# google/telluride_decoding

Hardware: AMD Instinct MI355X
Metric: TRF-fit samples/sec (higher is better)
Workload: dtype f32 (every product as 3 float16 products of a 2-piece split on the f16 MFMA, f32 accumulate, f64 slab sums; f64 solve)

## Files before the change

telluride_decoding_amd/csrc/lagcov.hip:

```cpp
#include <cstdlib>
#include <cstring>

#include "td_common.h"

namespace {

typedef float f32x16 __attribute__((ext_vector_type(16)));

constexpr int kThreads = 256;
constexpr int kTile = 128;
constexpr int kTileG = 64;
constexpr int kNpfU = 10;
constexpr int kNpfU2 = 13;
constexpr int kNpfG = 9;
constexpr int kLagsPerWg = 8;
constexpr int kHalo = 8;
constexpr size_t kLagcovScratchCap = size_t(256) << 20;

__device__ __forceinline__ int xcd_remap(int bid, int nwg) {
  const int q = nwg >> 3, r = nwg & 7;
  const int xcd = bid & 7, within = bid >> 3;
  const int base = xcd < r ? xcd * (q + 1) : r * (q + 1) + (xcd - r) * q;
  return base + within;
}

struct RowWindow {
  const float* base;
  int lo, hi;
  int ld, last;
};

__device__ __forceinline__ RowWindow row_window(const float* g, long long ld, long long row0,
                                                long long ut, long long valid, int c0, int c) {
  RowWindow rw;
  rw.base = g + (row0 + ut) * ld + c0;
  const long long lo = -ut, hi = valid - 1 - ut, lim = 1 << 20;
  rw.lo = (int)(lo < -lim ? -lim : (lo > lim ? lim : lo));
  rw.hi = (int)(hi < -lim ? -lim : (hi > lim ? lim : hi));
  rw.ld = (int)ld;
  rw.last = c - 1 - c0;
  return rw;
}

template <bool kVec4>
__device__ __forceinline__ float4 load_row4(const RowWindow& rw, int r, bool row_ok, int c4) {
  const int rc = max(rw.lo, min(r, rw.hi));
  const bool ok = row_ok && r >= rw.lo && r <= rw.hi;
  const float* p = rw.base + rc * rw.ld;
  float4 v;
  if (kVec4) {
    const bool ch_ok = c4 <= rw.last;
    v = *reinterpret_cast<const float4*>(p + (ch_ok ? c4 : 0));
    const bool k = ok && ch_ok;
    v.x = k ? v.x : 0.f; v.y = k ? v.y : 0.f; v.z = k ? v.z : 0.f; v.w = k ? v.w : 0.f;
  } else {
    const int last = rw.last;
    v.x = p[min(c4, last)]; v.y = p[min(c4 + 1, last)];
    v.z = p[min(c4 + 2, last)]; v.w = p[min(c4 + 3, last)];
    v.x = (ok && c4 + 0 <= last) ? v.x : 0.f;
    v.y = (ok && c4 + 1 <= last) ? v.y : 0.f;
    v.z = (ok && c4 + 2 <= last) ? v.z : 0.f;
    v.w = (ok && c4 + 3 <= last) ? v.w : 0.f;
  }
  return v;
}

template <bool kVec4>
__device__ __forceinline__ float4 load_row4_raw(const RowWindow& rw, int r, int c4) {
  const int rc = max(rw.lo, min(r, rw.hi));
  const float* p = rw.base + rc * rw.ld;
  float4 v;
  if (kVec4) {
    v = *reinterpret_cast<const float4*>(p + (c4 <= rw.last ? c4 : 0));
  } else {
    const int last = rw.last;
    v.x = p[min(c4, last)]; v.y = p[min(c4 + 1, last)];
    v.z = p[min(c4 + 2, last)]; v.w = p[min(c4 + 3, last)];
  }
  return v;
}

__device__ __forceinline__ float4 mask_row4(const RowWindow& rw, int r, bool row_ok, int c4, float4 v) {
  const bool ok = row_ok && r >= rw.lo && r <= rw.hi;
  v.x = (ok && c4 + 0 <= rw.last) ? v.x : 0.f;
  v.y = (ok && c4 + 1 <= rw.last) ? v.y : 0.f;
  v.z = (ok && c4 + 2 <= rw.last) ? v.z : 0.f;
  v.w = (ok && c4 + 3 <= rw.last) ? v.w : 0.f;
  return v;
}

template <bool kUnified, int kTileT, int kNPF, bool kVec4>
__device__ __forceinline__ void prefetch_tile(const LagParams& p, const LagWork& w, long long ut,
                                              int e0, int rows, int cat, int cbt, int tid,
                                              float4 (&pf)[kNPF]) {
  const int c4 = (tid & 15) * 4;
  const int r0 = tid >> 4;
  if (kUnified) {
    const RowWindow rw = row_window(p.a, p.lda, w.a_row0, ut, w.a_valid, cat * 64, p.ca);
#pragma unroll
    for (int i = 0; i < kNPF; ++i) {
      const int r = r0 + 16 * i;
      pf[i] = load_row4<kVec4>(rw, r, r < rows, c4);
    }
  } else {
    const RowWindow ra = row_window(p.a, p.lda, w.a_row0, ut, w.a_valid, cat * 64, p.ca);
    const RowWindow rb = row_window(p.b, p.ldb, w.b_row0, ut + e0, w.b_valid, cbt * 64, p.cb);
    const long long a_left = w.u_end - ut;
    const int a_lim = (int)(a_left < kTileT ? a_left : kTileT);
#pragma unroll
    for (int i = 0; i < kNPF; ++i) {
      const int r = r0 + 16 * i;
      if (16 * i + 15 < kTileT)
        pf[i] = load_row4<kVec4>(ra, r, r < a_lim, c4);
      else
        pf[i] = load_row4<kVec4>(rb, r - kTileT, r < rows, c4);
    }
  }
}

template <bool kUnified, int kTileT, int kNPF>
__device__ __forceinline__ void store_tile(float* lds, const LagWork& w, long long ut,
                                           int ones_col, int tid, float4 (&pf)[kNPF]) {
  const int c4 = (tid & 15) * 4;
#pragma unroll
  for (int i = 0; i < kNPF; ++i) {
    const int r = (tid >> 4) + 16 * i;
    float4 v = pf[i];
    if (!kUnified && 16 * i + 15 < kTileT && ones_col >= c4 && ones_col < c4 + 4) {
      const long long u = ut + r;
      const float one = (u >= w.u_begin && u < w.u_end) ? 1.f : 0.f;
      if (ones_col == c4) v.x = one;
      else if (ones_col == c4 + 1) v.y = one;
      else if (ones_col == c4 + 2) v.z = one;
      else v.w = one;
    }
    *reinterpret_cast<float4*>(lds + r * 64 + c4) = v;
  }
}

template <int kTileT, bool kM2, bool kN2>
__device__ __forceinline__ void mfma_tile(const float* __restrict__ as,
                                          const float* __restrict__ bs, int wave, int lane, int nk,
                                          f32x16 (&acc)[2][2][2]) {
  const int lr = lane & 31, lk = lane >> 5;
  const float* ap = as + lk * 64 + lr;
  const float* bp = bs + (lk + 2 * wave) * 64 + lr;
  auto ld = [&](int kk, float (&o)[6]) {
    o[0] = ap[kk * 128];
    o[1] = kM2 ? ap[kk * 128 + 32] : 0.f;
    o[2] = bp[kk * 128];
    o[3] = kN2 ? bp[kk * 128 + 32] : 0.f;
    o[4] = bp[kk * 128 + 64];
    o[5] = kN2 ? bp[kk * 128 + 96] : 0.f;
  };
  auto mm = [&](const float (&o)[6]) {
#pragma unroll
    for (int le = 0; le < 2; ++le) {
      const float b0 = o[2 + 2 * le], b1 = o[3 + 2 * le];
      acc[le][0][0] = __builtin_amdgcn_mfma_f32_32x32x2f32(o[0], b0, acc[le][0][0], 0, 0, 0);
      if (kM2) acc[le][1][0] = __builtin_amdgcn_mfma_f32_32x32x2f32(o[1], b0, acc[le][1][0], 0, 0, 0);
      if (kN2) {
        acc[le][0][1] = __builtin_amdgcn_mfma_f32_32x32x2f32(o[0], b1, acc[le][0][1], 0, 0, 0);
        if (kM2) acc[le][1][1] = __builtin_amdgcn_mfma_f32_32x32x2f32(o[1], b1, acc[le][1][1], 0, 0, 0);
      }
    }
  };
  const int nfull = nk >> 1;
  float c[6], n[6];
  ld(0, c);
  int kk = 0;
  for (; kk + 1 < nfull; kk += 2) {
    ld(kk + 1, n);
    mm(c);
    ld(kk + 2 < nfull ? kk + 2 : kk + 1, c);
    mm(n);
  }
  if (kk < nfull) mm(c);
  if (nk & 1) {
    ld(nfull, c);
    if (lk) { c[0] = 0.f; c[1] = 0.f; }
    mm(c);
  }
}

template <int kTileT, bool kM2, bool kN2>
__device__ __forceinline__ void mfma_tile_few(const float* __restrict__ as,
                                              const float* __restrict__ bs, int wave, int lane,
                                              int nk, int g, int lg, f32x16 (&acc)[2][2][2]) {
  const int lr = lane & 31, lk = lane >> 5;
  const int s_phases = 8 >> lg;
  const int nfull = nk >> 1;
#pragma unroll
  for (int le = 0; le < 2; ++le) {
    const int slot = 2 * wave + le;
    const int lag = slot & (g - 1), phase = slot >> lg;
    const float* ap = as + lk * 64 + lr;
    const float* bp = bs + (lk + lag) * 64 + lr;
    auto step = [&](int kk, bool tail) {
      const bool live = !tail || lk == 0;
      const float a0 = live ? ap[kk * 128] : 0.f;
      const float a1 = (kM2 && live) ? ap[kk * 128 + 32] : 0.f;
      const float b0 = bp[kk * 128];
      acc[le][0][0] = __builtin_amdgcn_mfma_f32_32x32x2f32(a0, b0, acc[le][0][0], 0, 0, 0);
      if (kM2) acc[le][1][0] = __builtin_amdgcn_mfma_f32_32x32x2f32(a1, b0, acc[le][1][0], 0, 0, 0);
      if (kN2) {
        const float b1 = bp[kk * 128 + 32];
        acc[le][0][1] = __builtin_amdgcn_mfma_f32_32x32x2f32(a0, b1, acc[le][0][1], 0, 0, 0);
        if (kM2) acc[le][1][1] = __builtin_amdgcn_mfma_f32_32x32x2f32(a1, b1, acc[le][1][1], 0, 0, 0);
      }
    };
#pragma unroll 4
    for (int kk = phase; kk < nfull; kk += s_phases) step(kk, false);
    if ((nk & 1) && (nfull & (s_phases - 1)) == phase) step(nfull, true);
  }
}

template <bool kUnified, int kTileT, int kNPF, bool kVec4, bool kFew>
__global__ __launch_bounds__(kThreads, 2) void lagcov_mfma_kernel(LagParams p) {
  extern __shared__ __attribute__((aligned(16))) float lds[];

  const int tid = threadIdx.x;
  const int lane = tid & 63;
  const int wave = __builtin_amdgcn_readfirstlane(tid >> 6);

  int id = xcd_remap(blockIdx.x, gridDim.x);
  const int group = id % p.n_groups; id /= p.n_groups;
  const int cbt = id % p.n_cbt; id /= p.n_cbt;
  const int cat = id % p.n_cat; id /= p.n_cat;
  const LagWork w = p.works[id];
  const int e0 = p.e_min + group * (kFew ? p.lag_g : kLagsPerWg);

  const int rows = kUnified ? kTileT + kHalo + e0 : 2 * kTileT + kHalo;
  const float* as = lds;
  const float* bs = kUnified ? lds + e0 * 64 : lds + kTileT * 64;

  const int ca_eff = p.ca + p.a_ones;
  const bool m2 = ca_eff - cat * 64 > 32;
  const bool n2 = p.cb - cbt * 64 > 32;
  const int ones_col = p.a_ones ? p.ca - cat * 64 : -1;

  f32x16 acc[2][2][2];
#pragma unroll
  for (int i = 0; i < 2; ++i)
#pragma unroll
    for (int j = 0; j < 2; ++j)
#pragma unroll
      for (int k = 0; k < 2; ++k)
#pragma unroll
        for (int r = 0; r < 16; ++r) acc[i][j][k][r] = 0.f;

  float4 pf[kNPF];
  prefetch_tile<kUnified, kTileT, kNPF, kVec4>(p, w, w.u_begin, e0, rows, cat, cbt, tid, pf);
  store_tile<kUnified, kTileT, kNPF>(lds, w, w.u_begin, ones_col, tid, pf);
  __syncthreads();

  for (long long ut = w.u_begin; ut < w.u_end; ut += kTileT) {
    const bool more = ut + kTileT < w.u_end;
    if (more)
      prefetch_tile<kUnified, kTileT, kNPF, kVec4>(p, w, ut + kTileT, e0, rows, cat, cbt, tid,
                                                      pf);
    const long long left = w.u_end - ut;
    const int nk = (kUnified && left < kTileT) ? (int)left : kTileT;
    if (kFew) {
      if (m2) {
        if (n2) mfma_tile_few<kTileT, true, true>(as, bs, wave, lane, nk, p.lag_g, p.lag_lg, acc);
        else    mfma_tile_few<kTileT, true, false>(as, bs, wave, lane, nk, p.lag_g, p.lag_lg, acc);
      } else {
        if (n2) mfma_tile_few<kTileT, false, true>(as, bs, wave, lane, nk, p.lag_g, p.lag_lg, acc);
        else    mfma_tile_few<kTileT, false, false>(as, bs, wave, lane, nk, p.lag_g, p.lag_lg, acc);
      }
    } else if (m2) {
      if (n2) mfma_tile<kTileT, true, true>(as, bs, wave, lane, nk, acc);
      else    mfma_tile<kTileT, true, false>(as, bs, wave, lane, nk, acc);
    } else {
      if (n2) mfma_tile<kTileT, false, true>(as, bs, wave, lane, nk, acc);
      else    mfma_tile<kTileT, false, false>(as, bs, wave, lane, nk, acc);
    }
    if (more) {
      __syncthreads();
      store_tile<kUnified, kTileT, kNPF>(lds, w, ut + kTileT, ones_col, tid, pf);
      __syncthreads();
    }
  }

  const int lr = lane & 31, lk = lane >> 5;
  float* slab = p.partial + (size_t)id * p.e_pad * p.ca_pad * p.cb_pad;
#pragma unroll
  for (int le = 0; le < 2; ++le) {
    int e_idx = group * kLagsPerWg + 2 * wave + le;
    if (kFew) {
      const int slot = 2 * wave + le;
      e_idx = ((slot >> p.lag_lg) * p.n_groups + group) * p.lag_g + (slot & (p.lag_g - 1));
    }
    float* pe = slab + (size_t)e_idx * p.ca_pad * p.cb_pad;
#pragma unroll
    for (int m = 0; m < 2; ++m)
#pragma unroll
      for (int n = 0; n < 2; ++n)
#pragma unroll
        for (int r = 0; r < 16; ++r) {
          const int i = cat * 64 + m * 32 + (r & 3) + 8 * (r >> 2) + 4 * lk;
          const int j = cbt * 64 + n * 32 + lr;
          pe[(size_t)i * p.cb_pad + j] = acc[le][m][n][r];
        }
  }
}

constexpr int kBfTile = 128;
template <int kRowDw, int kPieces> struct BfGeom {
  static constexpr int kRows = kRowDw == 83 ? 160 : 192;
  static constexpr int kPieceDw = 64 * kRowDw;
  static constexpr size_t kLdsBytes =
      sizeof(unsigned) * (2 * kPieces * kPieceDw + (kPieces == 2 ? 2 * 2 * 96 + 8 * 1024 : 0));
};
constexpr int kBfThreads = 512;

typedef td_u32x4 u32x4;

__device__ __forceinline__ float comp4(const float4& v, int q) {
  return q == 0 ? v.x : q == 1 ? v.y : q == 2 ? v.z : v.w;
}

template <bool kZero, int kBfPieceDw, bool kF16>
__device__ __forceinline__ void bf_kstep(const unsigned* __restrict__ ap,
                                         const unsigned* __restrict__ bp,
                                         const unsigned* a_mask, f32x16 (&acc)[4]) {
  constexpr int kP = kF16 ? 2 : 3;
  u32x4 a[kP];
  unsigned d[kP][6];
#pragma unroll
  for (int pc = 0; pc < kP; ++pc) {
#pragma unroll
    for (int i = 0; i < 4; ++i) a[pc][i] = ap[pc * kBfPieceDw + i];
#pragma unroll
    for (int i = 0; i < 6; ++i) d[pc][i] = bp[pc * kBfPieceDw + i];
  }
  if (a_mask) {
#pragma unroll
    for (int pc = 0; pc < kP; ++pc)
#pragma unroll
      for (int i = 0; i < 4; ++i) a[pc][i] &= a_mask[i];
  }
  u32x4 b[4][kP];
#pragma unroll
  for (int pc = 0; pc < kP; ++pc)
#pragma unroll
    for (int i = 0; i < 4; ++i) {
      b[0][pc][i] = d[pc][i];
      b[1][pc][i] = __builtin_amdgcn_alignbit(d[pc][i + 1], d[pc][i], 16);
      b[2][pc][i] = d[pc][i + 1];
      b[3][pc][i] = __builtin_amdgcn_alignbit(d[pc][i + 2], d[pc][i + 1], 16);
    }
  f32x16 c[4];
#pragma unroll
  for (int r = 0; r < 4; ++r) {
    if (kZero) {
#pragma unroll
      for (int k = 0; k < 16; ++k) c[r][k] = 0.f;
    } else {
      c[r] = acc[r];
    }
  }
  if constexpr (kF16) {
    constexpr int pa[3] = {1, 0, 0}, pb[3] = {0, 1, 0};
#pragma unroll
    for (int t = 0; t < 3; ++t)
#pragma unroll
      for (int r = 0; r < 4; ++r) c[r] = td_mfma_f16(a[pa[t] % kP], b[r][pb[t] % kP], c[r]);
  } else {
    constexpr int pa[6] = {2, 0, 1, 1, 0, 0}, pb[6] = {0, 2, 1, 0, 1, 0};
#pragma unroll
    for (int t = 0; t < 6; ++t)
#pragma unroll
      for (int r = 0; r < 4; ++r) c[r] = td_mfma_bf16(a[pa[t] % kP], b[r][pb[t] % kP], c[r]);
  }
#pragma unroll
  for (int r = 0; r < 4; ++r) acc[r] = c[r];
}

template <int kFrom, int kTo, int kBfPieceDw, bool kF16, int kChain>
__device__ __forceinline__ void bf_ksteps(const unsigned* __restrict__ ap,
                                          const unsigned* __restrict__ bp, f32x16 (&acc)[4],
                                          f32x16 (&total)[4]) {
#pragma unroll
  for (int s = kFrom; s < kTo; ++s) {
    if (s % kChain == 0) bf_kstep<true, kBfPieceDw, kF16>(ap + 8 * s, bp + 8 * s, nullptr, acc);
    else                 bf_kstep<false, kBfPieceDw, kF16>(ap + 8 * s, bp + 8 * s, nullptr, acc);
    if ((s + 1) % kChain == 0) {
#pragma unroll
      for (int r = 0; r < 4; ++r) total[r] += acc[r];
    }
    __builtin_amdgcn_sched_barrier(0);
  }
}

template <bool kVec4, int kBfRowDw, bool kF16, bool kVirt = false, bool kKs = false>
__global__ __launch_bounds__(kBfThreads) void lagcov_split_kernel(LagParams p) {
  static_assert(!kVirt || kF16, "virtual images: the float16 form");
  static_assert(!kKs || kVirt, "shared tasks: virtual images");
  constexpr int kChain = 8;
  constexpr int kP = kF16 ? 2 : 3;
  extern __shared__ __attribute__((aligned(16))) unsigned ldsu[];
  constexpr int kBfRows = BfGeom<kBfRowDw, kP>::kRows;
  constexpr int kBfPieceDw = BfGeom<kBfRowDw, kP>::kPieceDw;

  const int tid = threadIdx.x;
  const int lane = tid & 63;
  const int wave = __builtin_amdgcn_readfirstlane(tid >> 6);
  int quad = wave & 1, mt = (wave >> 1) & 1, nt = wave >> 2;

  int id = xcd_remap(blockIdx.x, gridDim.x);
  const int group = id % p.n_groups; id /= p.n_groups;
  const int part = id;
  LagWork w = p.works[id];
  const int e0 = group * kLagsPerWg;
  int lag_off = e0 + 4 * quad, out_lag = lag_off;
  bool active = true, a_ext = false;
  const VirtImage* img = nullptr;
  VirtSeg vs = {0, 0, 0};
  int kparts = 1, kq = 0;
  if constexpr (kVirt) {
    const VirtGroup* vg = p.vgroups + group;
    const VirtTask tk = vg->task[wave];
    img = p.vimgs + vg->image;
    mt = tk.mt; nt = tk.nt; lag_off = tk.lag0; out_lag = tk.out_lag;
    active = out_lag >= 0; a_ext = tk.a_ext != 0;
    if constexpr (kKs) {
      kparts = __builtin_amdgcn_readfirstlane((int)tk.kparts);
      kq = __builtin_amdgcn_readfirstlane((int)tk.kq);
    }
    vs = p.vsegs[id];
  }
  const int ksn = 8 / kparts, ks0 = kq * ksn;

  f32x16 total[4];
#pragma unroll
  for (int r = 0; r < 4; ++r)
#pragma unroll
    for (int k = 0; k < 16; ++k) total[r][k] = 0.f;

  const int c4 = (tid & 15) * 4, rg = tid >> 4;
  const bool has_tail = kBfRows == 192 || wave < 4;
  const bool early = wave < 4;
  float sc[4] = {1.f, 1.f, 1.f, 1.f};
  int vdesc[4] = {0, 0, 0, 0};
  if constexpr (kVirt) {
#pragma unroll
    for (int q = 0; q < 4; ++q) {
      const int k = kVec4 ? c4 + q : lane;
      vdesc[q] = (img->src[k] + 1) | (img->role[k] ? 0x100 : 0) | ((int)img->shift[k] << 16);
    }
  }
  constexpr int kVPairs = kBfRows / 16;
  auto v_src = [&](int q) { return (vdesc[q] & 0xff) - 1; };
  auto v_sh = [&](int q) { return vdesc[q] >> 16; };
  auto v_role = [&](int q) { return (vdesc[q] & 0x100) != 0; };
  if (kF16) {
#pragma unroll
    for (int q = 0; q < 4; ++q) {
      const int ch = kVirt ? v_src(q) : min(c4 + q, 63);
      const int k = ch >= 0 ? td_f16_scale_exp(td_chan_max_of(p.chan_max, ch)) : 0;
      sc[q] = __builtin_bit_cast(float, (unsigned)(127 + k) << 23);
      if (kVirt && ch < 0) sc[q] = 0.f;
    }
    if (blockIdx.x == 0 && tid < 128) {
      unsigned* all = const_cast<unsigned*>(p.chan_max);
      const unsigned m = td_chan_max_of(p.chan_max, tid);
      all[kChanShards * 128 + tid] = m;
      if (p.scale_out) p.scale_out[tid] = m;
    }
    if (p.zero_tab && blockIdx.x == (gridDim.x > 1 ? 1 : 0))
      for (int i = tid; i < kChanTab; i += kBfThreads) p.zero_tab[i] = 0u;
  }
  const bool never = false;
  float anchor_a = 0.f, anchor_b = 1.f;
  auto sched_anchor = [&](unsigned* dst) {
    if (!never || tid >= 160) return;
    reinterpret_cast<unsigned short*>(dst)[tid] = (unsigned short)(anchor_a * anchor_b);
  };
  float4 pf[6];
  auto interior = [&](long long ut) -> bool {
    return kVec4 && p.ca == 64 && ut >= 0 && ut + kBfRows <= w.a_valid;
  };
  auto vrange = [&](long long ut, int q, int& lo, int& hi) {
    const long long lim = 1 << 20;
    const long long a0 = -ut, b0 = w.a_valid - ut;
    const long long a1 = vs.seg_begin - ut, b1 = (vs.seg_end < w.a_valid ? vs.seg_end : w.a_valid) - ut;
    const int a0i = (int)(a0 < -lim ? -lim : (a0 > lim ? lim : a0)), b0i = (int)(b0 < -lim ? -lim : (b0 > lim ? lim : b0));
    const int a1i = (int)(a1 < -lim ? -lim : (a1 > lim ? lim : a1)), b1i = (int)(b1 < -lim ? -lim : (b1 > lim ? lim : b1));
    lo = (v_role(q) ? a1i : a0i) - v_sh(q);
    hi = (v_role(q) ? b1i : b0i) - v_sh(q);
    if (v_src(q) < 0) { lo = 0; hi = 0; }
  };
  int v_min_shift = 0, v_max_shift = 0;
  bool v_any_role1 = false;
  if constexpr (kVirt) { v_min_shift = img->min_shift; v_max_shift = img->max_shift; v_any_role1 = img->any_role1 != 0; }
  auto vinside = [&](long long ut) -> bool {
    const long long lo = v_any_role1 && vs.seg_begin > 0 ? vs.seg_begin : 0;
    const long long hi = v_any_role1 && vs.seg_end < w.a_valid ? vs.seg_end : w.a_valid;
    return ut + v_min_shift >= lo && ut + kBfRows + v_max_shift <= hi;
  };
  auto prefetch_to = [&](long long ut, float4 (&pfr)[6]) {
    if constexpr (kVirt) {
      if (vinside(ut)) {
        const int ld = (int)p.lda;
        const float* base = p.a + (w.a_row0 + ut) * p.lda;
        if (kVec4) {
          const int off = (4 * rg + v_sh(0)) * ld + (v_src(0) < 0 ? 0 : v_src(0));
#pragma unroll
          for (int s = 0; s < 4; ++s) pfr[s] = *reinterpret_cast<const float4*>(base + s * ld + off);
          if (has_tail) {
            const float* tb = base + kBfTile * ld;
            const int toff = off - 2 * rg * ld;
#pragma unroll
            for (int s = 0; s < 2; ++s) pfr[4 + s] = *reinterpret_cast<const float4*>(tb + s * ld + toff);
          }
        } else {
          const int off = (2 * wave + v_sh(0)) * ld + (v_src(0) < 0 ? 0 : v_src(0));
          float* pv = reinterpret_cast<float*>(&pfr[0]);
#pragma unroll
          for (int j = 0; j < kVPairs; ++j) {
            pv[2 * j] = (base + 16 * j * ld)[off];
            pv[2 * j + 1] = (base + (16 * j + 1) * ld)[off];
          }
        }
        return;
      }
      const float* base = p.a + (w.a_row0 + ut) * p.lda;
      const int ld = (int)p.lda;
      const long long l0 = -ut, h0 = w.a_valid - 1 - ut, lim = 1 << 20;
      const int rlo = (int)(l0 < -lim ? -lim : (l0 > lim ? lim : l0));
      const int rhi = (int)(h0 < -lim ? -lim : (h0 > lim ? lim : h0));
      if (kVec4) {
        const int src = v_src(0) < 0 ? 0 : v_src(0), sh = v_sh(0);
#pragma unroll
        for (int s = 0; s < 4; ++s) {
          const int rc = max(rlo, min(4 * rg + s + sh, rhi));
          pfr[s] = *reinterpret_cast<const float4*>(base + rc * ld + src);
        }
        if (has_tail) {
#pragma unroll
          for (int s = 0; s < 2; ++s) {
            const int rc = max(rlo, min(kBfTile + 2 * rg + s + sh, rhi));
            pfr[4 + s] = *reinterpret_cast<const float4*>(base + rc * ld + src);
          }
        }
      } else {
        const int src = v_src(0) < 0 ? 0 : v_src(0), sh = v_sh(0);
        float* pv = reinterpret_cast<float*>(&pfr[0]);
#pragma unroll
        for (int j = 0; j < 2 * kVPairs; ++j) {
          const int r = 16 * (j >> 1) + 2 * wave + (j & 1);
          const int rc = max(rlo, min(r + sh, rhi));
          pv[j] = base[rc * ld + src];
        }
      }
      return;
    }
    if (interior(ut)) {
      const float* base = p.a + (w.a_row0 + ut) * p.lda + c4;
      const int ld = (int)p.lda;
#pragma unroll
      for (int s = 0; s < 4; ++s)
        pfr[s] = *reinterpret_cast<const float4*>(base + (4 * rg + s) * ld);
      if (has_tail) {
#pragma unroll
        for (int s = 0; s < 2; ++s)
          pfr[4 + s] = *reinterpret_cast<const float4*>(base + (kBfTile + 2 * rg + s) * ld);
      }
      return;
    }
    const RowWindow rw = row_window(p.a, p.lda, w.a_row0, ut, w.a_valid, 0, p.ca);
#pragma unroll
    for (int s = 0; s < 4; ++s) pfr[s] = load_row4_raw<kVec4>(rw, 4 * rg + s, c4);
    if (has_tail) {
#pragma unroll
      for (int s = 0; s < 2; ++s) pfr[4 + s] = load_row4_raw<kVec4>(rw, kBfTile + 2 * rg + s, c4);
    }
  };
  auto prefetch = [&](long long ut) { prefetch_to(ut, pf); };
  auto store_from = [&](long long ut, unsigned* buf, const float4 (&pfr)[6]) {
    if constexpr (kVirt && !kVec4) {
      const float* pv = reinterpret_cast<const float*>(&pfr[0]);
      unsigned* dst = buf + lane * kBfRowDw + wave;
      if (vinside(ut)) {
#pragma unroll
        for (int j = 0; j < kVPairs; ++j) {
          unsigned h, l;
          td_split2_f16(pv[2 * j] * sc[0], pv[2 * j + 1] * sc[0], h, l);
          dst[8 * j] = h;
          dst[kBfPieceDw + 8 * j] = l;
        }
        return;
      }
      int lo, hi;
      vrange(ut, 0, lo, hi);
#pragma unroll
      for (int j = 0; j < kVPairs; ++j) {
        const int r = 16 * j + 2 * wave;
        const float x0 = (r >= lo && r < hi) ? pv[2 * j] : 0.f;
        const float x1 = (r + 1 >= lo && r + 1 < hi) ? pv[2 * j + 1] : 0.f;
        unsigned h, l;
        td_split2_f16(x0 * sc[0], x1 * sc[0], h, l);
        dst[8 * j] = h;
        dst[kBfPieceDw + 8 * j] = l;
      }
      return;
    }
    float4 v[6];
#pragma unroll
    for (int s = 0; s < 6; ++s) v[s] = pfr[s];
    if constexpr (kVirt) {
      if (!vinside(ut))
#pragma unroll
      for (int q = 0; q < 4; ++q) {
        int lo, hi;
        vrange(ut, kVec4 ? 0 : q, lo, hi);
        if (lo <= 0 && hi >= kBfRows) continue;
#pragma unroll
        for (int s = 0; s < 4; ++s) {
          const int r = 4 * rg + s;
          float& x = reinterpret_cast<float*>(&v[s])[q];
          x = (r >= lo && r < hi) ? x : 0.f;
        }
#pragma unroll
        for (int s = 0; s < 2; ++s) {
          const int r = kBfTile + 2 * rg + s;
          float& x = reinterpret_cast<float*>(&v[4 + s])[q];
          x = (r >= lo && r < hi) ? x : 0.f;
        }
      }
    } else
    if (!interior(ut)) {
      const RowWindow rw = row_window(p.a, p.lda, w.a_row0, ut, w.a_valid, 0, p.ca);
#pragma unroll
      for (int s = 0; s < 4; ++s) v[s] = mask_row4(rw, 4 * rg + s, true, c4, pfr[s]);
      if (has_tail) {
#pragma unroll
        for (int s = 0; s < 2; ++s) v[4 + s] = mask_row4(rw, kBfTile + 2 * rg + s, true, c4, pfr[4 + s]);
      }
    }
#pragma unroll
    for (int q = 0; q < 4; ++q) {
      unsigned* dst = buf + (c4 + q) * kBfRowDw + 2 * rg;
      if (kF16) {
        unsigned h[2], l[2];
#pragma unroll
        for (int d = 0; d < 2; ++d)
          td_split2_f16(comp4(v[2 * d], q) * sc[q], comp4(v[2 * d + 1], q) * sc[q], h[d], l[d]);
        dst[0] = h[0]; dst[1] = h[1];
        dst[kBfPieceDw] = l[0]; dst[kBfPieceDw + 1] = l[1];
      } else {
        unsigned h[2], m[2], l[2];
#pragma unroll
        for (int d = 0; d < 2; ++d)
          td_split3(comp4(v[2 * d], q), comp4(v[2 * d + 1], q), h[d], m[d], l[d]);
        dst[0] = h[0]; dst[1] = h[1];
        dst[kBfPieceDw] = m[0]; dst[kBfPieceDw + 1] = m[1];
        dst[(kP - 1) * kBfPieceDw] = l[0]; dst[(kP - 1) * kBfPieceDw + 1] = l[1];
      }
    }
    if (has_tail) {
#pragma unroll
      for (int q = 0; q < 4; ++q) {
        unsigned* tail = buf + (c4 + q) * kBfRowDw + kBfTile / 2 + rg;
        if (kF16) {
          unsigned h, l;
          td_split2_f16(comp4(v[4], q) * sc[q], comp4(v[5], q) * sc[q], h, l);
          tail[0] = h;
          tail[kBfPieceDw] = l;
        } else {
          unsigned h, m, l;
          td_split3(comp4(v[4], q), comp4(v[5], q), h, m, l);
          tail[0] = h;
          tail[kBfPieceDw] = m;
          tail[(kP - 1) * kBfPieceDw] = l;
        }
      }
    }
  };
  auto store = [&](long long ut, unsigned* buf) { store_from(ut, buf, pf); };

  const int lj = lane & 31, lg = lane >> 5;
  const int a_off = (mt * 32 + lj) * kBfRowDw + 4 * lg;
  const int b_off = (nt * 32 + lj) * kBfRowDw + 4 * lg + (lag_off >> 1);

  f32x16 acc[4];
  unsigned* const buf0 = ldsu;
  unsigned* const buf1 = ldsu + kP * kBfPieceDw;
  for (; id < p.n_work; id += p.n_part) {
  if (id != part) {
    __syncthreads();
    w = p.works[id];
    if constexpr (kVirt) vs = p.vsegs[id];
  }
  if constexpr (kKs) {
    const long long u_stop = vs.u_end_ext;
    float4 pf2[6];
    prefetch_to(w.u_begin, pf);
    store_from(w.u_begin, buf0, pf);
    if (w.u_begin + kBfTile < u_stop) prefetch_to(w.u_begin + kBfTile, pf);
    __syncthreads();
    auto ks_tile = [&](long long ut, const unsigned* cur, unsigned* nxt, float4 (&pfa)[6], float4 (&pfb)[6]) {
      const bool more = ut + kBfTile < u_stop;
      if (ut + 2 * kBfTile < u_stop) prefetch_to(ut + 2 * kBfTile, pfb);
      long long left = (a_ext ? u_stop : w.u_end) - ut;
      if (!active) left = 0;
      const unsigned* ap = cur + a_off;
      const unsigned* bp = cur + b_off;
      if (left >= kBfTile) {
        bf_kstep<true, kBfPieceDw, kF16>(ap + 8 * ks0, bp + 8 * ks0, nullptr, acc);
        for (int s = ks0 + 1; s < ks0 + ksn; ++s)
          bf_kstep<false, kBfPieceDw, kF16>(ap + 8 * s, bp + 8 * s, nullptr, acc);
#pragma unroll
        for (int r = 0; r < 4; ++r) total[r] += acc[r];
      } else if (left > 16 * ks0) {
        const int nk = (int)left;
#pragma unroll
        for (int r = 0; r < 4; ++r)
#pragma unroll
          for (int k = 0; k < 16; ++k) acc[r][k] = 0.f;
        const int t_hi = min(nk, 16 * (ks0 + ksn));
        for (int t0 = 16 * ks0; t0 < t_hi; t0 += 16) {
          const int cnt = nk - t0 - 8 * lg;
          unsigned mask[4];
#pragma unroll
          for (int d = 0; d < 4; ++d)
            mask[d] = cnt >= 2 * d + 2 ? 0xffffffffu : cnt == 2 * d + 1 ? 0x0000ffffu : 0u;
          bf_kstep<false, kBfPieceDw, kF16>(ap + (t0 >> 1), bp + (t0 >> 1), mask, acc);
        }
#pragma unroll
        for (int r = 0; r < 4; ++r) total[r] += acc[r];
      }
      if (more) {
        store_from(ut + kBfTile, nxt, pfa);
        __syncthreads();
      }
    };
    for (long long ut = w.u_begin; ut < u_stop; ut += 2 * kBfTile) {
      ks_tile(ut, buf0, buf1, pf, pf2);
      if (ut + kBfTile < u_stop) ks_tile(ut + kBfTile, buf1, buf0, pf2, pf);
    }
    continue;
  }
  prefetch(w.u_begin);
  store(w.u_begin, buf0);
  __syncthreads();

  const long long u_stop = kVirt ? vs.u_end_ext : w.u_end;
  int parity = 0;
  for (long long ut = w.u_begin; ut < u_stop; ut += kBfTile, parity ^= 1) {
    const unsigned* cur = parity ? buf1 : buf0;
    unsigned* nxt = parity ? buf0 : buf1;
    const bool more = ut + kBfTile < u_stop;
    if (more) prefetch(ut + kBfTile);
    long long left = w.u_end - ut;
    if constexpr (kVirt) {
      if (a_ext) left = u_stop - ut;
      if (!active) left = 0;
      if (left < kBfTile && more) store(ut + kBfTile, nxt);
    }
    const unsigned* ap = cur + a_off;
    const unsigned* bp = cur + b_off;
    if (left >= kBfTile) {
      bf_ksteps<0, 2, kBfPieceDw, kF16, kChain>(ap, bp, acc, total);
      if (more && early) { store(ut + kBfTile, nxt); sched_anchor(nxt); }
      bf_ksteps<2, 6, kBfPieceDw, kF16, kChain>(ap, bp, acc, total);
      if (more && !early) { store(ut + kBfTile, nxt); sched_anchor(nxt); }
      bf_ksteps<6, 8, kBfPieceDw, kF16, kChain>(ap, bp, acc, total);
    } else {
      const int nk = (int)left;
#pragma unroll
      for (int r = 0; r < 4; ++r)
#pragma unroll
        for (int k = 0; k < 16; ++k) acc[r][k] = 0.f;
      for (int t0 = 0; t0 < nk; t0 += 16) {
        const int cnt = nk - t0 - 8 * lg;
        unsigned mask[4];
#pragma unroll
        for (int d = 0; d < 4; ++d)
          mask[d] = cnt >= 2 * d + 2 ? 0xffffffffu : cnt == 2 * d + 1 ? 0x0000ffffu : 0u;
        bf_kstep<false, kBfPieceDw, kF16>(ap + (t0 >> 1), bp + (t0 >> 1), mask, acc);
      }
#pragma unroll
      for (int r = 0; r < 4; ++r) total[r] += acc[r];
    }
    if (more) __syncthreads();
  }
  }

  if constexpr (kKs) {
    float* const red = reinterpret_cast<float*>(ldsu);
    const int task = wave / kparts;
    for (int step = kparts >> 1; step >= 1; step >>= 1) {
      __syncthreads();
      if (kq >= step && kq < 2 * step) {
        float* dst = red + (size_t)(task * step + kq - step) * 4096 + lane;
#pragma unroll
        for (int r = 0; r < 4; ++r)
#pragma unroll
          for (int k = 0; k < 16; ++k) dst[(r * 16 + k) * 64] = total[r][k];
      }
      __syncthreads();
      if (kq < step) {
        const float* src = red + (size_t)(task * step + kq) * 4096 + lane;
#pragma unroll
        for (int r = 0; r < 4; ++r)
#pragma unroll
          for (int k = 0; k < 16; ++k) total[r][k] += src[(r * 16 + k) * 64];
      }
    }
    active = active && kq == 0;
  }
  if constexpr (kVirt) {
    if (active) {
      float* slab = p.partial + (size_t)part * p.slab_elems;
      const int lr = lane & 31, lk = lane >> 5;
#pragma unroll
      for (int r = 0; r < 4; ++r) {
        float* pe = slab + (size_t)(out_lag + r) * 1024;
#pragma unroll
        for (int k = 0; k < 16; ++k) pe[((k & 3) + 8 * (k >> 2) + 4 * lk) * 32 + lr] = total[r][k];
      }
    }
    return;
  }
  float* slab = p.partial + (size_t)part * p.e_pad * p.ca_pad * p.cb_pad;
#pragma unroll
  for (int r = 0; r < 4; ++r) {
    float* pe = slab + (size_t)(e0 + 4 * quad + r) * p.ca_pad * p.cb_pad;
    const int lr = lane & 31, lk = lane >> 5;
#pragma unroll
    for (int k = 0; k < 16; ++k) {
      const int i = mt * 32 + (k & 3) + 8 * (k >> 2) + 4 * lk;
      const int j = nt * 32 + lr;
      pe[(size_t)i * p.cb_pad + j] = total[r][k];
    }
  }
}

struct Narrow16Params {
  const float* x;
  const float* y;
  long long ldx, ldy;
  int c, d, pre, l1;
  const LagWork* works;
  int n_lg, lpw;
  int do_main, do_tgt;
  float* part;
  float* tpart;
  double* csum;
  double* ysum;
  long long n_part;
};

typedef float n16_f32x4 __attribute__((ext_vector_type(4)));

__device__ __forceinline__ float n16_load(__amdgpu_buffer_rsrc_t rs, unsigned voff) {
  return __builtin_bit_cast(float, __builtin_amdgcn_raw_buffer_load_b32(rs, (int)voff, 0, 0));
}

template <bool kMain, bool kTgt, int kLpw, int kD, bool kPre>
__global__ __launch_bounds__(256) void lagcov_narrow16_kernel(Narrow16Params p) {
  const int tid = threadIdx.x, lane = tid & 63;
  const int wave = __builtin_amdgcn_readfirstlane(tid >> 6);
  const int g = wave % p.n_lg, sub = wave / p.n_lg, n_sub = 4 / p.n_lg;
  const LagWork w = p.works[blockIdx.x];
  const long long len = w.u_end - w.u_begin;
  const long long sub_len = ((len + n_sub - 1) / n_sub + 3) / 4 * 4;
  const long long ub = w.u_begin + sub * sub_len;
  const long long ue = ub + sub_len < w.u_end ? ub + sub_len : w.u_end;
  const int j = lane & 15, k = lane >> 4;
  const int e0 = g * kLpw;
  const int ne = p.l1 - e0 < kLpw ? p.l1 - e0 : kLpw;
  const __amdgpu_buffer_rsrc_t rx = __builtin_amdgcn_make_buffer_rsrc(
      const_cast<float*>(p.x + w.b_row0 * p.ldx), 0,
      w.b_valid > 0 ? (int)(((w.b_valid - 1) * p.ldx + p.c) * 4) : 0, 0x00020000);
  const __amdgpu_buffer_rsrc_t ry = __builtin_amdgcn_make_buffer_rsrc(
      const_cast<float*>(p.y + w.a_row0 * p.ldy), 0,
      w.a_valid > 0 ? (int)(((w.a_valid - 1) * p.ldy + p.d) * 4) : 0, 0x00020000);
  const unsigned row_x = (unsigned)(p.ldx * 4), row_y = (unsigned)(p.ldy * 4);
  const unsigned lane_x = j < p.c ? (unsigned)k * row_x + 4u * j : 0x80000000u;
  const unsigned lane_y = (unsigned)k * row_y;
  const unsigned lag0 = (unsigned)e0 * row_x, pre_x = (unsigned)p.pre * row_x;
  n16_f32x4 acc[kLpw];
  float tacc[kD][kLpw];
#pragma unroll
  for (int q = 0; q < kLpw; ++q) {
    acc[q] = n16_f32x4{0.f, 0.f, 0.f, 0.f};
#pragma unroll
    for (int col = 0; col < kD; ++col) tacc[col][q] = 0.f;
  }
  float cs = 0.f, ys[kD];
#pragma unroll
  for (int col = 0; col < kD; ++col) ys[col] = 0.f;
  constexpr int kU = kLpw >= 8 ? 2 : 4;
  for (long long u = ub; u < ue; u += 4 * kU) {
    const unsigned vx = lane_x + (unsigned)u * row_x;
    const unsigned vy = lane_y + (unsigned)u * row_y;
    float a[kU], b[kU][kLpw], bt[kU][kLpw], yv[kU][kD];
#pragma unroll
    for (int st = 0; st < kU; ++st) {
      const unsigned vs = vx + (unsigned)(4 * st) * row_x;
      a[st] = n16_load(rx, vs);
#pragma unroll
      for (int q = 0; q < kLpw; ++q) b[st][q] = n16_load(rx, vs + lag0 + (unsigned)q * row_x);
      if (kTgt) {
#pragma unroll
        for (int col = 0; col < kD; ++col) yv[st][col] = n16_load(ry, vy + (unsigned)(4 * st) * row_y + 4u * col);
        if (kPre) {
#pragma unroll
          for (int q = 0; q < kLpw; ++q) bt[st][q] = n16_load(rx, vs + lag0 + (unsigned)q * row_x - pre_x);
        }
      }
    }
#pragma unroll
    for (int st = 0; st < kU; ++st) {
      const bool in_slab = k + 4 * st < ue - u;
      const float av = in_slab ? a[st] : 0.f;
#pragma unroll
      for (int q = 0; q < kLpw; ++q) {
        if (kMain) acc[q] = __builtin_amdgcn_mfma_f32_16x16x4f32(av, b[st][q], acc[q], 0, 0, 0);
        if (kTgt) {
#pragma unroll
          for (int col = 0; col < kD; ++col) {
            const float yc = in_slab ? yv[st][col] : 0.f;
            tacc[col][q] += yc * (kPre ? bt[st][q] : b[st][q]);
          }
        }
      }
      if (kTgt) {
        cs += av;
#pragma unroll
        for (int col = 0; col < kD; ++col) ys[col] += in_slab ? yv[st][col] : 0.f;
      }
    }
  }
  constexpr int kSlot = kLpw * 256 + kD * kLpw * 16 + 16 + 16;
  __shared__ float red[3 * kSlot];
  if (kTgt) {
#pragma unroll
    for (int col = 0; col < kD; ++col) {
#pragma unroll
      for (int q = 0; q < kLpw; ++q) {
        float t = tacc[col][q];
        t += __shfl_xor(t, 16);
        t += __shfl_xor(t, 32);
        tacc[col][q] = t;
      }
      float t = ys[col];
      t += __shfl_xor(t, 16);
      t += __shfl_xor(t, 32);
      ys[col] = t;
    }
    cs += __shfl_xor(cs, 16);
    cs += __shfl_xor(cs, 32);
  }
  if (sub > 0) {
    float* slot = red + ((sub - 1) * p.n_lg + g) * kSlot;
    if (kMain) {
#pragma unroll
      for (int q = 0; q < kLpw; ++q)
#pragma unroll
        for (int r = 0; r < 4; ++r) slot[(q * 4 + r) * 64 + lane] = acc[q][r];
    }
    if (kTgt && k == 0) {
#pragma unroll
      for (int col = 0; col < kD; ++col) {
#pragma unroll
        for (int q = 0; q < kLpw; ++q) slot[kLpw * 256 + (col * kLpw + q) * 16 + j] = tacc[col][q];
        if (j == 0) slot[kLpw * 256 + kD * kLpw * 16 + 16 + col] = ys[col];
      }
      slot[kLpw * 256 + kD * kLpw * 16 + j] = cs;
    }
  }
  __syncthreads();
  if (sub > 0) return;
  for (int o = 1; o < n_sub; ++o) {
    const float* slot = red + ((o - 1) * p.n_lg + g) * kSlot;
    if (kMain) {
#pragma unroll
      for (int q = 0; q < kLpw; ++q)
#pragma unroll
        for (int r = 0; r < 4; ++r) acc[q][r] += slot[(q * 4 + r) * 64 + lane];
    }
    if (kTgt && k == 0) {
#pragma unroll
      for (int col = 0; col < kD; ++col) {
#pragma unroll
        for (int q = 0; q < kLpw; ++q) tacc[col][q] += slot[kLpw * 256 + (col * kLpw + q) * 16 + j];
        ys[col] += slot[kLpw * 256 + kD * kLpw * 16 + 16 + col];
      }
      cs += slot[kLpw * 256 + kD * kLpw * 16 + j];
    }
  }
  const long long pidx = blockIdx.x;
  if (kMain) {
#pragma unroll
    for (int q = 0; q < kLpw; ++q) {
      if (q < ne) {
        float* dst = p.part + ((size_t)pidx * p.l1 + (e0 + q)) * 256 + (4 * k) * 16 + j;
#pragma unroll
        for (int r = 0; r < 4; ++r) dst[r * 16] = acc[q][r];
      }
    }
  }
  if (!kTgt || k != 0) return;
#pragma unroll
  for (int col = 0; col < kD; ++col) {
    if (col < p.d) {
#pragma unroll
      for (int q = 0; q < kLpw; ++q)
        if (q < ne) p.tpart[(((size_t)col * p.n_part + pidx) * p.l1 + (e0 + q)) * 16 + j] = tacc[col][q];
      if (g == 0 && j == 0) p.ysum[(size_t)col * p.n_part + pidx] = (double)ys[col];
    }
  }
  if (g == 0) p.csum[pidx * 16 + j] = (double)cs;
}

__global__ __launch_bounds__(256) void chan_max_kernel(const float* __restrict__ x, long long ld,
                                                       int c, long long row0, long long row1,
                                                       unsigned* __restrict__ tab, int vec4) {
  __shared__ unsigned red[16][64];
  const int tid = threadIdx.x, c4 = (tid & 15) * 4, rl = tid >> 4;
  unsigned m[4] = {0u, 0u, 0u, 0u};
  const long long stride = (long long)gridDim.x * 16;
  if (vec4) {
    if (c4 < c) {
      long long r = row0 + (long long)blockIdx.x * 16 + rl;
      for (; r + 3 * stride < row1; r += 4 * stride) {
        float4 v[4];
#pragma unroll
        for (int k = 0; k < 4; ++k) v[k] = *reinterpret_cast<const float4*>(x + (r + k * stride) * ld + c4);
#pragma unroll
        for (int k = 0; k < 4; ++k) {
          m[0] = max(m[0], __float_as_uint(v[k].x) & 0x7fffffffu);
          m[1] = max(m[1], __float_as_uint(v[k].y) & 0x7fffffffu);
          m[2] = max(m[2], __float_as_uint(v[k].z) & 0x7fffffffu);
          m[3] = max(m[3], __float_as_uint(v[k].w) & 0x7fffffffu);
        }
      }
      for (; r < row1; r += stride) {
        const float4 v = *reinterpret_cast<const float4*>(x + r * ld + c4);
        m[0] = max(m[0], __float_as_uint(v.x) & 0x7fffffffu);
        m[1] = max(m[1], __float_as_uint(v.y) & 0x7fffffffu);
        m[2] = max(m[2], __float_as_uint(v.z) & 0x7fffffffu);
        m[3] = max(m[3], __float_as_uint(v.w) & 0x7fffffffu);
      }
    }
  } else {
    for (long long r = row0 + (long long)blockIdx.x * 16 + rl; r < row1; r += stride)
#pragma unroll
      for (int q = 0; q < 4; ++q)
        if (c4 + q < c) m[q] = max(m[q], __float_as_uint(x[r * ld + c4 + q]) & 0x7fffffffu);
  }
#pragma unroll
  for (int q = 0; q < 4; ++q) red[rl][c4 + q] = m[q];
  __syncthreads();
  if (tid < 64) {
    unsigned t = 0u;
#pragma unroll
    for (int k = 0; k < 16; ++k) t = max(t, red[k][tid]);
    if (tid < c && t) atomicMax(tab + (blockIdx.x % kChanShards) * 128 + tid, t);
  }
}

__global__ __launch_bounds__(256) void chan_max_wide_kernel(const float* __restrict__ x, long long ld, int c,
                                                            long long row0, long long row1,
                                                            unsigned* __restrict__ tab, int vec4) {
  __shared__ unsigned red[8][128];
  const int tid = threadIdx.x, c4 = (tid & 31) * 4, rl = tid >> 5;
  unsigned m[4] = {0u, 0u, 0u, 0u};
  const long long stride = (long long)gridDim.x * 8;
  long long r = row0 + (long long)blockIdx.x * 8 + rl;
  if (vec4) {
    if (c4 < c) {
      for (; r + 3 * stride < row1; r += 4 * stride) {
        float4 v[4];
#pragma unroll
        for (int k = 0; k < 4; ++k) v[k] = *reinterpret_cast<const float4*>(x + (r + k * stride) * ld + c4);
#pragma unroll
        for (int k = 0; k < 4; ++k) {
          m[0] = max(m[0], __float_as_uint(v[k].x) & 0x7fffffffu);
          m[1] = max(m[1], __float_as_uint(v[k].y) & 0x7fffffffu);
          m[2] = max(m[2], __float_as_uint(v[k].z) & 0x7fffffffu);
          m[3] = max(m[3], __float_as_uint(v[k].w) & 0x7fffffffu);
        }
      }
      for (; r < row1; r += stride) {
        const float4 v = *reinterpret_cast<const float4*>(x + r * ld + c4);
        m[0] = max(m[0], __float_as_uint(v.x) & 0x7fffffffu);
        m[1] = max(m[1], __float_as_uint(v.y) & 0x7fffffffu);
        m[2] = max(m[2], __float_as_uint(v.z) & 0x7fffffffu);
        m[3] = max(m[3], __float_as_uint(v.w) & 0x7fffffffu);
      }
    }
  } else {
    const int ch = tid & 127, rh = tid >> 7;
    unsigned mm = 0u;
    const long long st2 = (long long)gridDim.x * 2;
    long long rr = row0 + (long long)blockIdx.x * 2 + rh;
    if (ch < c) {
      for (; rr + 3 * st2 < row1; rr += 4 * st2) {
        float v[4];
#pragma unroll
        for (int k = 0; k < 4; ++k) v[k] = x[(rr + k * st2) * ld + ch];
#pragma unroll
        for (int k = 0; k < 4; ++k) mm = max(mm, __float_as_uint(v[k]) & 0x7fffffffu);
      }
      for (; rr < row1; rr += st2) mm = max(mm, __float_as_uint(x[rr * ld + ch]) & 0x7fffffffu);
    }
#pragma unroll
    for (int k = 0; k < 8; ++k) red[k][ch] = 0u;
    __syncthreads();
    atomicMax(&red[0][ch], mm);
    __syncthreads();
    if (tid < 128 && tid < c && red[0][tid]) atomicMax(tab + (blockIdx.x % kChanShards) * 128 + tid, red[0][tid]);
    return;
  }
#pragma unroll
  for (int q = 0; q < 4; ++q) red[rl][c4 + q] = m[q];
  __syncthreads();
  if (tid < 128) {
    unsigned t = 0u;
#pragma unroll
    for (int k = 0; k < 8; ++k) t = max(t, red[k][tid]);
    if (tid < c && t) atomicMax(tab + (blockIdx.x % kChanShards) * 128 + tid, t);
  }
}

__global__ __launch_bounds__(256) void bf16_mfma_probe_kernel(const unsigned* __restrict__ ops,
                                                              float* __restrict__ out, int iters) {
  u32x4 a[3], b[3];
// ... 2477 lines not shown
```

Baseline: 1.155 billion.

## Hand-schedule f16 split k-step in inline asm with skewed lag assignment

For the non-virtual float16 split kernel, replaces the compiler-generated k-step with an inline-assembly sequence that does explicit LDS reads, alignbit shifts to derive lag+1 B operands, and an interleaved MFMA schedule over hard-coded VGPRs. Each wave now covers lags {+0,+1,+4,+5} instead of four consecutive lags, so the shifted B fragments can be reused across lag pairs, and the output write is remapped to match. It also drops the per-tile register copy of the prefetched rows. This trades compiler register allocation for fixed clobbered VGPRs and manual waitcnt/nop handling, which risks register pressure and hazards.

```diff
diff --git a/telluride_decoding_amd/csrc/lagcov.hip b/telluride_decoding_amd/csrc/lagcov.hip
--- a/telluride_decoding_amd/csrc/lagcov.hip
+++ b/telluride_decoding_amd/csrc/lagcov.hip
@@ -321,10 +321,110 @@
   return q == 0 ? v.x : q == 1 ? v.y : q == 2 ? v.z : v.w;
 }
 
-template <bool kZero, int kBfPieceDw, bool kF16>
+#define TD_KS_C0(r) "0"
+#define TD_KS_C1(r) "%" #r
+#define TD_KS_BODY(C, MASK_L, MASK_H, TAIL)                                              \
+  "ds_read2_b32 v[224:225], %[bp0] offset0:%[o0] offset1:%[o1]\n"                        \
+  "ds_read2_b32 v[226:227], %[bp0] offset0:%[o2] offset1:%[o3]\n"                        \
+  "ds_read2_b32 v[228:229], %[bp0] offset0:%[o4] offset1:%[o5]\n"                        \
+  "ds_read_b32 v230, %[bp0] offset:%[ob]\n"                                              \
+  "ds_read2_b32 v[220:221], %[ap1] offset0:%[o0] offset1:%[o1]\n"                        \
+  "ds_read2_b32 v[222:223], %[ap1] offset0:%[o2] offset1:%[o3]\n"                        \
+  "ds_read2_b32 v[232:233], %[bp1] offset0:%[o0] offset1:%[o1]\n"                        \
+  "ds_read2_b32 v[234:235], %[bp1] offset0:%[o2] offset1:%[o3]\n"                        \
+  "ds_read2_b32 v[236:237], %[bp1] offset0:%[o4] offset1:%[o5]\n"                        \
+  "ds_read_b32 v238, %[bp1] offset:%[ob]\n"                                              \
+  "ds_read2_b32 v[216:217], %[ap0] offset0:%[o0] offset1:%[o1]\n"                        \
+  "ds_read2_b32 v[218:219], %[ap0] offset0:%[o2] offset1:%[o3]\n"                        \
+  "s_waitcnt lgkmcnt(6)\n"                                                               \
+  MASK_L                                                                                 \
+  "v_alignbit_b32 v240, v225, v224, 16\n"                                                \
+  "v_alignbit_b32 v241, v226, v225, 16\n"                                                \
+  "v_alignbit_b32 v242, v227, v226, 16\n"                                                \
+  "v_alignbit_b32 v243, v228, v227, 16\n"                                                \
+  "v_alignbit_b32 v244, v229, v228, 16\n"                                                \
+  "v_alignbit_b32 v245, v230, v229, 16\n"                                                \
+  "v_mfma_f32_32x32x16_f16 %0, v[220:223], v[224:227], " C(0) "\n"                       \
+  "s_waitcnt lgkmcnt(0)\n"                                                               \
+  MASK_H                                                                                 \
+  "v_alignbit_b32 v248, v233, v232, 16\n"                                                \
+  "v_alignbit_b32 v249, v234, v233, 16\n"                                                \
+  "v_mfma_f32_32x32x16_f16 %1, v[220:223], v[240:243], " C(1) "\n"                       \
+  "v_alignbit_b32 v250, v235, v234, 16\n"                                                \
+  "v_alignbit_b32 v251, v236, v235, 16\n"                                                \
+  "v_mfma_f32_32x32x16_f16 %2, v[220:223], v[226:229], " C(2) "\n"                       \
+  "v_alignbit_b32 v252, v237, v236, 16\n"                                                \
+  "v_alignbit_b32 v253, v238, v237, 16\n"                                                \
+  "v_mfma_f32_32x32x16_f16 %3, v[220:223], v[242:245], " C(3) "\n"                       \
+  "v_mfma_f32_32x32x16_f16 %0, v[216:219], v[232:235], %0\n"                             \
+  "v_mfma_f32_32x32x16_f16 %1, v[216:219], v[248:251], %1\n"                             \
+  "v_mfma_f32_32x32x16_f16 %2, v[216:219], v[234:237], %2\n"                             \
+  "v_mfma_f32_32x32x16_f16 %3, v[216:219], v[250:253], %3\n"                             \
+  "v_mfma_f32_32x32x16_f16 %0, v[216:219], v[224:227], %0\n"                             \
+  "v_mfma_f32_32x32x16_f16 %1, v[216:219], v[240:243], %1\n"                             \
+  "v_mfma_f32_32x32x16_f16 %2, v[216:219], v[226:229], %2\n"                             \
+  "v_mfma_f32_32x32x16_f16 %3, v[216:219], v[242:245], %3\n"                             \
+  TAIL
+#define TD_KS_MASK_L                                                                     \
+  "v_and_b32 v220, %[m0], v220\n" "v_and_b32 v221, %[m1], v221\n"                        \
+  "v_and_b32 v222, %[m2], v222\n" "v_and_b32 v223, %[m3], v223\n"
+#define TD_KS_MASK_H                                                                     \
+  "v_and_b32 v216, %[m0], v216\n" "v_and_b32 v217, %[m1], v217\n"                        \
+  "v_and_b32 v218, %[m2], v218\n" "v_and_b32 v219, %[m3], v219\n"
+#define TD_KS_TAIL "s_nop 15\ns_nop 3\n"
+#define TD_KS_INS                                                                        \
+  [ap0] "v"(ap0), [ap1] "v"(ap1), [bp0] "v"(bp0), [bp1] "v"(bp1),                        \
+  [o0] "n"(kOff), [o1] "n"(kOff + 1), [o2] "n"(kOff + 2), [o3] "n"(kOff + 3),            \
+  [o4] "n"(kOff + 4), [o5] "n"(kOff + 5), [ob] "n"(4 * (kOff + 6)),                      \
+  [m0] "v"(m0), [m1] "v"(m1), [m2] "v"(m2), [m3] "v"(m3)
+#define TD_KS_CLOBBER                                                                    \
+  "memory", "v216", "v217", "v218", "v219", "v220", "v221", "v222", "v223", "v224", "v225", "v226", "v227", \
+  "v228", "v229", "v230", "v231", "v232", "v233", "v234", "v235", "v236", "v237", "v238", "v239", "v240",   \
+  "v241", "v242", "v243", "v244", "v245", "v246", "v247", "v248", "v249", "v250", "v251", "v252", "v253",   \
+  "v254", "v255"
+#define TD_KS_ASM(OUT, C, ML, MH, TAIL)                                                  \
+  asm volatile(TD_KS_BODY(C, ML, MH, TAIL)                                               \
+               : OUT(acc[0]), OUT(acc[1]), OUT(acc[2]), OUT(acc[3]) : TD_KS_INS : TD_KS_CLOBBER)
+
+__device__ __forceinline__ unsigned lds_addr(const unsigned* p) {
+  return (unsigned)(size_t)(__attribute__((address_space(3))) const unsigned*)p;
+}
+
+template <bool kZero, bool kMask, bool kLast, int kOff>
+__device__ __forceinline__ void bf_kstep_skip(unsigned ap0, unsigned ap1, unsigned bp0, unsigned bp1,
+                                              const unsigned* a_mask, f32x16 (&acc)[4]) {
+  unsigned m0 = 0, m1 = 0, m2 = 0, m3 = 0;
+  if constexpr (kMask) { m0 = a_mask[0]; m1 = a_mask[1]; m2 = a_mask[2]; m3 = a_mask[3]; }
+  if constexpr (kZero) {
+    if constexpr (kMask) {
+      if constexpr (kLast) TD_KS_ASM("=&v", TD_KS_C0, TD_KS_MASK_L, TD_KS_MASK_H, TD_KS_TAIL);
+      else TD_KS_ASM("=&v", TD_KS_C0, TD_KS_MASK_L, TD_KS_MASK_H, "");
+    } else {
+      if constexpr (kLast) TD_KS_ASM("=&v", TD_KS_C0, "", "", TD_KS_TAIL);
+      else TD_KS_ASM("=&v", TD_KS_C0, "", "", "");
+    }
+  } else {
+    if constexpr (kMask) {
+      if constexpr (kLast) TD_KS_ASM("+v", TD_KS_C1, TD_KS_MASK_L, TD_KS_MASK_H, TD_KS_TAIL);
+      else TD_KS_ASM("+v", TD_KS_C1, TD_KS_MASK_L, TD_KS_MASK_H, "");
+    } else {
+      if constexpr (kLast) TD_KS_ASM("+v", TD_KS_C1, "", "", TD_KS_TAIL);
+      else TD_KS_ASM("+v", TD_KS_C1, "", "", "");
+    }
+  }
+}
+
+template <bool kZero, int kBfPieceDw, bool kF16, bool kSkip = false, int kOff = 0, bool kLast = true>
 __device__ __forceinline__ void bf_kstep(const unsigned* __restrict__ ap,
                                          const unsigned* __restrict__ bp,
                                          const unsigned* a_mask, f32x16 (&acc)[4]) {
+  if constexpr (kSkip) {
+    static_assert(kF16, "lags +0, +1, +4, +5: the float16 form");
+    const unsigned a0 = lds_addr(ap), b0 = lds_addr(bp);
+    if (a_mask) bf_kstep_skip<kZero, true, kLast, kOff>(a0, a0 + 4 * kBfPieceDw, b0, b0 + 4 * kBfPieceDw, a_mask, acc);
+    else bf_kstep_skip<kZero, false, kLast, kOff>(a0, a0 + 4 * kBfPieceDw, b0, b0 + 4 * kBfPieceDw, a_mask, acc);
+    return;
+  }
   constexpr int kP = kF16 ? 2 : 3;
   u32x4 a[kP];
   unsigned d[kP][6];
@@ -378,10 +478,23 @@
   for (int r = 0; r < 4; ++r) acc[r] = c[r];
 }
 
-template <int kFrom, int kTo, int kBfPieceDw, bool kF16, int kChain>
+template <int kFrom, int kTo, int kBfPieceDw, bool kF16, int kChain, bool kSkip = false>
 __device__ __forceinline__ void bf_ksteps(const unsigned* __restrict__ ap,
                                           const unsigned* __restrict__ bp, f32x16 (&acc)[4],
                                           f32x16 (&total)[4]) {
+  if constexpr (kSkip) {
+    if constexpr (kFrom < kTo) {
+      constexpr bool kLast = (kFrom + 1) % kChain == 0;
+      bf_kstep<kFrom % kChain == 0, kBfPieceDw, kF16, true, 8 * kFrom, kLast>(ap, bp, nullptr, acc);
+      if (kLast) {
+#pragma unroll
+        for (int r = 0; r < 4; ++r) total[r] += acc[r];
+      }
+      __builtin_amdgcn_sched_barrier(0);
+      bf_ksteps<kFrom + 1, kTo, kBfPieceDw, kF16, kChain, true>(ap, bp, acc, total);
+    }
+    return;
+  }
 #pragma unroll
   for (int s = kFrom; s < kTo; ++s) {
     if (s % kChain == 0) bf_kstep<true, kBfPieceDw, kF16>(ap + 8 * s, bp + 8 * s, nullptr, acc);
@@ -408,13 +521,14 @@
   const int lane = tid & 63;
   const int wave = __builtin_amdgcn_readfirstlane(tid >> 6);
   int quad = wave & 1, mt = (wave >> 1) & 1, nt = wave >> 2;
+  constexpr bool kSkip = kF16 && !kVirt;
 
   int id = xcd_remap(blockIdx.x, gridDim.x);
   const int group = id % p.n_groups; id /= p.n_groups;
   const int part = id;
   LagWork w = p.works[id];
   const int e0 = group * kLagsPerWg;
-  int lag_off = e0 + 4 * quad, out_lag = lag_off;
+  int lag_off = e0 + (kSkip ? 2 : 4) * quad, out_lag = lag_off;
   bool active = true, a_ext = false;
   const VirtImage* img = nullptr;
   VirtSeg vs = {0, 0, 0};
@@ -607,9 +721,12 @@
       }
       return;
     }
-    float4 v[6];
-#pragma unroll
-    for (int s = 0; s < 6; ++s) v[s] = pfr[s];
+    float4 vcopy[6];
+    float4 (&v)[6] = kSkip ? const_cast<float4 (&)[6]>(pfr) : vcopy;
+    if constexpr (!kSkip) {
+#pragma unroll
+      for (int s = 0; s < 6; ++s) vcopy[s] = pfr[s];
+    }
     if constexpr (kVirt) {
       if (!vinside(ut))
 #pragma unroll
@@ -763,11 +880,11 @@
     const unsigned* ap = cur + a_off;
     const unsigned* bp = cur + b_off;
     if (left >= kBfTile) {
-      bf_ksteps<0, 2, kBfPieceDw, kF16, kChain>(ap, bp, acc, total);
+      bf_ksteps<0, 2, kBfPieceDw, kF16, kChain, kSkip>(ap, bp, acc, total);
       if (more && early) { store(ut + kBfTile, nxt); sched_anchor(nxt); }
-      bf_ksteps<2, 6, kBfPieceDw, kF16, kChain>(ap, bp, acc, total);
+      bf_ksteps<2, 6, kBfPieceDw, kF16, kChain, kSkip>(ap, bp, acc, total);
       if (more && !early) { store(ut + kBfTile, nxt); sched_anchor(nxt); }
-      bf_ksteps<6, 8, kBfPieceDw, kF16, kChain>(ap, bp, acc, total);
+      bf_ksteps<6, 8, kBfPieceDw, kF16, kChain, kSkip>(ap, bp, acc, total);
     } else {
       const int nk = (int)left;
 #pragma unroll
@@ -780,7 +897,7 @@
 #pragma unroll
         for (int d = 0; d < 4; ++d)
           mask[d] = cnt >= 2 * d + 2 ? 0xffffffffu : cnt == 2 * d + 1 ? 0x0000ffffu : 0u;
-        bf_kstep<false, kBfPieceDw, kF16>(ap + (t0 >> 1), bp + (t0 >> 1), mask, acc);
+        bf_kstep<false, kBfPieceDw, kF16, kSkip>(ap + (t0 >> 1), bp + (t0 >> 1), mask, acc);
       }
 #pragma unroll
       for (int r = 0; r < 4; ++r) total[r] += acc[r];
@@ -828,7 +945,8 @@
   float* slab = p.partial + (size_t)part * p.e_pad * p.ca_pad * p.cb_pad;
 #pragma unroll
   for (int r = 0; r < 4; ++r) {
-    float* pe = slab + (size_t)(e0 + 4 * quad + r) * p.ca_pad * p.cb_pad;
+    const int lag = kSkip ? out_lag + (r & 1) + 4 * (r >> 1) : out_lag + r;
+    float* pe = slab + (size_t)lag * p.ca_pad * p.cb_pad;
     const int lr = lane & 31, lk = lane >> 5;
 #pragma unroll
     for (int k = 0; k < 16; ++k) {
```

Measured after the change: 1.183 billion (median of 6 runs). +2.4%, better.
